# youmi-zym/TemporalStereo

Measured on AMD Instinct MI355X. Metric: stereo pairs/sec, FlyingThings3D 540x960 D=192 (aggregation hot path), higher is better.
Workload: dtype f32

## Files before the change

### include/ts_hip.h

```cpp
#ifndef TS_HIP_H
#define TS_HIP_H

#include <stddef.h>
#include <stdint.h>

#ifdef __cplusplus
extern "C" {
#endif

#define TS_OK 0
#define TS_ERR_NULL (-1)
#define TS_ERR_SHAPE (-2)
#define TS_ERR_UNSUPPORTED (-3)
#define TS_ERR_ALIGN (-4)

int ts_version(void);
const char* ts_last_error_string(void);

size_t ts_block_cost_workspace_bytes(int B, int C, int H, int W, int D, int scales);

int ts_block_cost_int_fwd(const float* left, const float* right, float* out, void* workspace,
                          int B, int C, int H, int W, int D, int scales, void* stream);

int ts_block_cost_sampled_fwd(const float* left, const float* right, const float* disp, float* out,
// ... 167 lines not shown
int ts_conv3d_hw_x6_fwd(const float* x, const void* w6, const float* scale, const float* shift, float* y,
                        int B, int Cin, int Cout, int D, int H, int W, int dilation, int act, float act_param,
                        long long in_bstride, long long in_cstride, long long out_bstride, long long out_cstride,
                        const float* addend, long long addend_bstride, void* workspace, size_t workspace_bytes, void* stream);
typedef struct ts_peer_ctx {
  void* region[8];
  int rank, world;
} ts_peer_ctx;
size_t ts_peer_region_bytes(void);
int ts_peer_max_floats(void);
int ts_peer_max_ranks(void);
int ts_peer_alloc(void** region, void* handle64);
int ts_peer_open(const void* handle64, void** region);
int ts_peer_close(void* region);
int ts_peer_free(void* region);
int ts_peer_status(const void* ctx, int* status, void* stream);
int ts_peer_status_async(const void* ctx, int* host_status, void* stream);
long long ts_peer_set_timeout_ms(long long ms);
int ts_peer_reset(const void* ctx, void* stream);
int ts_peer_all_gather(const void* ctx, const float* src, float* dst, int n, void* stream);
int ts_peer_all_reduce_sum(const void* ctx, float* buf, int n, const float* scale, void* stream);

int ts_conv3d_hw_x6s_supported(int Cin, int Cout, int H, int W, int mode);
size_t ts_conv3d_hw_x6s_weight_bytes(int Cin, int Cout, int mode);
int ts_conv3d_hw_x6s_weight_split(const float* w_t, void* w6, int Cin, int Cout, int w_pad, int mode, void* stream);
int ts_conv3d_hw_x6s_fwd(const float* x, const void* w6, const float* scale, const float* shift, float* y,
                         int B, int Cin, int Cout, int D, int H, int W, int mode, int act, float act_param,
                         long long in_bstride, long long in_cstride, long long out_bstride, long long out_cstride, void* stream);
int ts_conv3d_d_fwd(const float* x, const float* w_t, const float* scale, const float* shift, float* y,
                    int B, int Cin, int Cout, int Din, int H, int W, int k, int stride, int dilation,
                    int padding, int transposed, int act, float act_param,
                    long long in_bstride, long long in_cstride, long long out_bstride,
                    long long out_cstride, void* stream);
size_t ts_conv3d_bwd_weight_workspace_bytes(int Cin, int Cout, int taps);
int ts_conv3d_hw_bwd_data(const float* dy, const float* w_b, float* dx, int B, int Cin, int Cout, int D, int H, int W,
                          int stride, int dilation, int transposed, long long dy_bstride, long long dy_cstride,
                          long long dx_bstride, long long dx_cstride, void* stream);
int ts_conv3d_hw_bwd_weight(const float* x, const float* dy, float* dw, int B, int Cin, int Cout, int D, int H, int W,
                            int stride, int dilation, long long x_bstride, long long x_cstride, long long dy_bstride,
                            long long dy_cstride, void* workspace, size_t workspace_bytes, void* stream);
int ts_conv3d_d_bwd_data(const float* dy, const float* w_b, float* dx, int B, int Cin, int Cout, int Din, int H, int W,
                         int k, int stride, int dilation, int padding, int transposed, long long dy_bstride,
                         long long dy_cstride, long long dx_bstride, long long dx_cstride, void* stream);
int ts_conv3d_d_bwd_weight(const float* x, const float* dy, float* dw, int B, int Cin, int Cout, int Din, int H, int W,
                           int k, int stride, int dilation, int padding, long long x_bstride, long long x_cstride,
                           long long dy_bstride, long long dy_cstride, void* workspace, size_t workspace_bytes,
                           void* stream);
int ts_resize3d_add_act_fwd(const float* a, const float* add, float* out, int B, int C, int Da, int Ha, int Wa,
                            int D, int H, int W, int act, long long a_bstride, long long a_cstride,
                            long long add_bstride, long long add_cstride, long long out_bstride,
                            long long out_cstride, void* stream);
int ts_pool3d5_avgmax_fwd(const float* x, float* out_avg, float* out_max, int B, int C, int D, int H, int W,
                          long long x_bstride, long long x_cstride, long long avg_bstride, long long avg_cstride,
                          long long max_bstride, long long max_cstride, void* stream);
int ts_merge_candidates_fwd(const float* volume, const float* sample, const float* mem_sample, const float* mem_cost,
                            const float* past_w, const float* past_scale, const float* past_shift,
                            float* out_sample, float* out_volume, int B, int C, int D0, int K, int H, int W,
                            long long vol_bstride, long long vol_cstride, long long out_bstride,
                            long long out_cstride, void* stream);
int ts_convex_upsample_fwd(const float* mask, const float* disp, float* out, int B, int H, int W, int factor,
                           float disp_scale, void* stream);
int ts_convex_upsample_candidates_fwd(const float* mask, const float* disp, float* out, float* low, float* high,
                                      float* candidates, int B, int H, int W, int factor, float disp_scale, float range,
                                      int channel_offset, int channels_total, void* stream);
int ts_unet_upsample_fwd(const float* mask, const float* disp, float* out, int B, int h, int w, int Ho, int Wo,
                         void* stream);
// ... 59 lines not shown
```

### temporalstereo_amd/_lib.py

```python
import ctypes
import os
import threading

_HERE = os.path.dirname(os.path.abspath(__file__))
LIB_PATH = os.path.join(_HERE, "libts_hip.so")

_lock = threading.Lock()
_lib = None

c_f32p = ctypes.c_void_p
c_ptr = ctypes.c_void_p
c_int = ctypes.c_int
c_size = ctypes.c_size_t
c_float = ctypes.c_float

SIGNATURES = {
    "ts_version": (c_int, []),
    "ts_last_error_string": (ctypes.c_char_p, []),
    "ts_block_cost_workspace_bytes": (c_size, [c_int] * 6),
    "ts_block_cost_int_fwd": (c_int, [c_f32p, c_f32p, c_f32p, c_ptr] + [c_int] * 6 + [c_ptr]),
    "ts_block_cost_sampled_fwd": (c_int, [c_f32p, c_f32p, c_f32p, c_f32p, c_ptr] + [c_int] * 6 + [c_ptr]),
    "ts_block_cost_sampled_warped_fwd": (c_int, [c_f32p, c_f32p, c_f32p, c_f32p, c_ptr] + [c_int] * 6 + [c_ptr]),
    "ts_block_cost_sampled_corr_fwd": (c_int, [c_f32p, c_f32p, c_f32p, c_f32p, c_ptr] + [c_int] * 6 + [c_ptr]),
    "ts_conv3d_hw_warp_workspace_bytes": (c_size, [c_int] * 5),
# ... 60 lines not shown
    "ts_peer_status_async": (c_int, [c_ptr, c_ptr, c_ptr]),
    "ts_peer_set_timeout_ms": (ctypes.c_longlong, [ctypes.c_longlong]),
    "ts_peer_reset": (c_int, [c_ptr, c_ptr]),
    "ts_peer_all_gather": (c_int, [c_ptr, c_f32p, c_f32p, c_int, c_ptr]),
    "ts_peer_all_reduce_sum": (c_int, [c_ptr, c_f32p, c_int, c_f32p, c_ptr]),
    "ts_conv_weight_layout": (c_int, [c_f32p, c_f32p] + [c_int] * 4 + [ctypes.c_longlong] * 3 + [c_int, c_ptr]),
    "ts_conv_weight_layout_many": (c_int, [c_ptr, c_int, c_int, c_ptr]),
    "ts_conv_weight_layout_many2": (c_int, [c_ptr, c_int, c_int, c_ptr]),
    "ts_conv_wgrad_defer": (c_int, [c_int]),
    "ts_conv_wgrad_pending": (c_int, []),
    "ts_conv_wgrad_take": (c_int, [c_ptr, c_size, ctypes.POINTER(c_int), ctypes.POINTER(c_int)]),
    "ts_conv_wgrad_finish_many": (c_int, [c_ptr, c_int, c_int, c_ptr]),
    "ts_conv_set_chunk_cap": (c_int, [c_int]),
    "ts_conv3d_hw_x6_supported": (c_int, [c_int] * 6),
    "ts_conv3d_hw_x6_weight_bytes": (ctypes.c_size_t, [c_int] * 2),
    "ts_conv3d_hw_x6_weight_split": (c_int, [c_f32p, c_ptr, c_int, c_int, c_ptr]),
    "ts_conv3d_hw_x6_weight_split_from": (c_int, [c_f32p, c_ptr, c_int, c_int] + [ctypes.c_longlong] * 3 + [c_int, c_ptr]),
    "ts_conv3d_hw_x6_workspace_bytes": (c_size, [c_int] * 6),
    "ts_conv3d_hw_x6s_supported": (c_int, [c_int] * 5),
    "ts_conv3d_hw_x6s_weight_bytes": (c_size, [c_int] * 3),
    "ts_conv3d_hw_x6s_weight_split": (c_int, [c_f32p, c_ptr, c_int, c_int, c_int, c_int, c_ptr]),
    "ts_conv3d_hw_x6s_fwd": (c_int, [c_f32p, c_ptr, c_f32p, c_f32p, c_f32p] + [c_int] * 8 + [c_float] + [ctypes.c_longlong] * 4 + [c_ptr]),
    "ts_conv3d_hw_x6_fwd": (c_int, [c_f32p, c_ptr, c_f32p, c_f32p, c_f32p] + [c_int] * 8 + [c_float] + [ctypes.c_longlong] * 4 +
                            [c_f32p, ctypes.c_longlong, c_ptr, c_size, c_ptr]),
    "ts_conv3d_hw_fwd": (c_int, [c_f32p] * 5 + [c_int] * 10 + [c_float] + [ctypes.c_longlong] * 4 +
                         [c_f32p, ctypes.c_longlong, c_ptr, c_size, c_ptr]),
    "ts_conv3d_hw_workspace_bytes": (c_size, [c_int] * 8),
    "ts_conv3d_hw_bwd_data": (c_int, [c_f32p] * 3 + [c_int] * 9 + [ctypes.c_longlong] * 4 + [c_ptr]),
    "ts_conv3d_bwd_weight_workspace_bytes": (ctypes.c_size_t, [c_int] * 3),
    "ts_conv3d_hw_bwd_weight": (c_int, [c_f32p] * 3 + [c_int] * 8 + [ctypes.c_longlong] * 4 + [c_ptr, ctypes.c_size_t, c_ptr]),
    "ts_conv3d_d_bwd_data": (c_int, [c_f32p] * 3 + [c_int] * 11 + [ctypes.c_longlong] * 4 + [c_ptr]),
    "ts_conv3d_d_bwd_weight": (c_int, [c_f32p] * 3 + [c_int] * 10 + [ctypes.c_longlong] * 4 + [c_ptr, ctypes.c_size_t, c_ptr]),
    "ts_conv3d_d_fwd": (c_int, [c_f32p] * 5 + [c_int] * 12 + [c_float] + [ctypes.c_longlong] * 4 + [c_ptr]),
    "ts_resize3d_add_act_fwd": (c_int, [c_f32p] * 3 + [c_int] * 9 + [ctypes.c_longlong] * 6 + [c_ptr]),
    "ts_pool3d5_avgmax_fwd": (c_int, [c_f32p] * 3 + [c_int] * 5 + [ctypes.c_longlong] * 6 + [c_ptr]),
    "ts_merge_candidates_fwd": (c_int, [c_f32p] * 9 + [c_int] * 6 + [ctypes.c_longlong] * 4 + [c_ptr]),
    "ts_convex_upsample_fwd": (c_int, [c_f32p] * 3 + [c_int] * 4 + [c_float, c_ptr]),
    "ts_convex_upsample_candidates_fwd": (c_int, [c_f32p] * 6 + [c_int] * 4 + [c_float, c_float, c_int, c_int, c_ptr]),
    "ts_unet_upsample_fwd": (c_int, [c_f32p] * 3 + [c_int] * 5 + [c_ptr]),
    "ts_convex_upsample_bwd": (c_int, [c_f32p] * 5 + [c_int] * 4 + [c_float, c_ptr]),
    "ts_unet_upsample_bwd": (c_int, [c_f32p] * 5 + [c_ptr] + [c_int] * 5 + [c_ptr]),
    "ts_deconv2d_k4s2_fwd": (c_int, [c_f32p] * 5 + [c_int] * 6 + [ctypes.c_longlong, c_ptr]),
    "ts_resize_bilinear_fwd": (c_int, [c_f32p] * 2 + [c_int] * 6 + [c_float, ctypes.c_longlong, c_ptr]),
    "ts_resize_bilinear_pair_fwd": (c_int, [c_f32p] * 4 + [c_int] * 6 + [c_float, c_float, c_ptr]),
    "ts_range_candidates_fwd": (c_int, [c_f32p] * 4 + [c_int] * 3 + [c_float, c_int, c_int, c_ptr]),
    "ts_project_to_3d_fwd": (c_int, [c_f32p] * 7 + [c_int] * 6 + [c_float, c_ptr]),
    "ts_reproject_memory_workspace_bytes": (c_size, [c_int] * 5),
    "ts_reproject_memory_fwd": (c_int, [c_f32p, ctypes.c_longlong, c_int, c_int, c_f32p, c_f32p, c_int, c_f32p, c_int, c_int,
                                        c_f32p, c_int, c_f32p, c_f32p, c_f32p, c_float, c_float, c_f32p, c_f32p, c_f32p,
                                        c_ptr, c_int, c_int, c_int, c_ptr]),
    "ts_resize3d_add_act_bwd": (c_int, [c_f32p] * 5 + [c_int] * 9 + [c_ptr]),
    "ts_pool3d5_avgmax_bwd": (c_int, [c_f32p] * 4 + [c_int] * 5 + [c_ptr]),
    "ts_merge_candidates_bwd": (c_int, [c_f32p] * 5 + [c_int] * 5 + [c_ptr]),
    "ts_copy_rows_fwd": (c_int, [c_f32p] * 2 + [ctypes.c_longlong] * 4 + [c_ptr]),
    "ts_plan_create": (c_ptr, []),
    "ts_plan_destroy": (None, [c_ptr]),
    "ts_plan_length": (c_int, [c_ptr]),
    "ts_plan_add_call": (c_int, [c_ptr, ctypes.c_char_p, ctypes.POINTER(ctypes.c_ulonglong), c_int]),
    "ts_plan_run": (c_int, [c_ptr]),
    "ts_stream_fork": (c_int, [c_ptr, c_ptr]),
    "ts_event_record": (c_int, [c_int, c_ptr]),
    "ts_event_wait": (c_int, [c_int, c_ptr]),
}

_QUERIES = frozenset(n for n in SIGNATURES if n.endswith("_bytes") or n.startswith("ts_plan_") or
                     n in ("ts_version", "ts_last_error_string", "ts_conv_cout_pad", "ts_conv3d_hw_x6_supported", "ts_conv3d_hw_x6s_supported", "ts_peer_max_floats", "ts_peer_max_ranks",
                           "ts_peer_alloc", "ts_peer_open", "ts_peer_close", "ts_peer_free", "ts_peer_status", "ts_peer_status_async",
                           "ts_peer_set_timeout_ms", "ts_peer_reset", "ts_bn_set_small_elems",
                           "ts_conv_wgrad_defer", "ts_conv_wgrad_pending", "ts_conv_wgrad_take"))


def lib():
    rec = getattr(_tls, "recorder", None)
    if rec is not None:
        return rec.proxy
    return _real_lib()


def _real_lib():
    global _lib
    if _lib is None:
        with _lock:
            if _lib is None:
                if not os.path.exists(LIB_PATH):
                    raise RuntimeError(
                        "temporalstereo_amd: %s is missing -- build it with "
                        "`python -m temporalstereo_amd.build` (there is no fallback path)" % LIB_PATH)
                handle = ctypes.CDLL(LIB_PATH)
                for name, (res, args) in SIGNATURES.items():
                    fn = getattr(handle, name, None)
                    if fn is None:
                        raise RuntimeError("libts_hip.so does not export %s (stale build?)" % name)
                    fn.restype = res
                    fn.argtypes = args
                _lib = handle
    return _lib


_tls = threading.local()
# ... 105 lines not shown
```

### temporalstereo_amd/aggregation/native.py

```python
import os
import time

import torch
import torch.nn as nn

from .. import _lib
from .. import functional as TF

ACT_NONE, ACT_SILU, ACT_RELU, ACT_TANH_OFFSET, ACT_HEAD_PAIR = 0, 1, 2, 3, 4


def _stream():
    return _lib.current_stream_handle()


_PAR = {"on": False, "aux": None, "kinds": frozenset(__import__("os").environ.get("TS_BRANCHES", "hourglass").split(","))}


def _aux_stream():
    return _PAR["aux"]


_STAGE_CAP = int(os.environ.get("TS_STAGE_CHUNK_CAP", "8"))

# ... 290 lines not shown
        if getattr(f, "_tape", None) is not None:
            f._tape.splits.append((f, "x6", 0))
    return w6


X6S = os.environ.get("TS_CONV_X6S", "1") != "0"
_X6S_MIN_GRID = int(os.environ.get("TS_CONV_X6S_MIN_GRID", "256"))
_X6S_MIN_GRID_T3 = int(os.environ.get("TS_CONV_X6S_MIN_GRID_T3", "400"))
X6S_S2, X6S_T3, X6S_T4 = 0, 1, 2


def x6s_weights(f, mode):
    w6 = getattr(f, "w6s", None)
    if w6 is None:
        L = _lib._real_lib()
        w6 = torch.empty(int(L.ts_conv3d_hw_x6s_weight_bytes(f.cin, f.cout, mode)), device=f.w.device, dtype=torch.uint8)
        _lib.check(L.ts_conv3d_hw_x6s_weight_split(f.w.data_ptr(), w6.data_ptr(), f.cin, f.cout, f.w.shape[2], mode, _stream()),
                   "ts_conv3d_hw_x6s_weight_split")
        f.w6s = w6
        f.w6s_mode = mode
        if getattr(f, "_tape", None) is not None:
            f._tape.splits.append((f, "x6s", mode))
    elif getattr(f, "w6s_mode", mode) != mode:
        raise RuntimeError("x6s_weights: this layer's weights were split for mode %d, asked for mode %d" % (f.w6s_mode, mode))
    return w6


def x6s_grid(B, cout, D, H, W, mode):
    if mode == X6S_S2:
        return ((((H - 1) // 2 + 1) + 3) // 4) * ((((W - 1) // 2 + 1) + 31) // 32) * D * B * ((cout + 31) // 32)
    return ((H + 7) // 8) * ((W + 31) // 32) * D * B * ((cout + 15) // 16)


def conv_hw(x, f, stride=1, dilation=1, transposed=False, out=None, act=None, act_param=0.0, addend=None, second=None,
            out_second=None):
    B, Cin, D, H, W = x.shape
    if second is not None:
        if B != 1 or second.shape != x.shape or _strides5(second)[1] != _strides5(x)[1]:
            raise ValueError("conv_hw(second=...): two tensors of one shape and channel stride with batch 1")
        if (second.data_ptr() - x.data_ptr()) % 4:
            raise ValueError("conv_hw(second=...): allocations are not 4-byte aligned relative to each other")
        B = 2
    assert Cin == f.cin, (Cin, f.cin)
    if transposed:
        Ho, Wo = 2 * H, 2 * W
    else:
        Ho = (H + 2 * dilation - 2 * dilation - 1) // stride + 1
        Wo = (W + 2 * dilation - 2 * dilation - 1) // stride + 1
    if out is None:
        out = torch.empty((B, f.cout, D, Ho, Wo), device=x.device, dtype=torch.float32)
    ib, ic = _strides5(x)
    if second is not None:
        ib = (second.data_ptr() - x.data_ptr()) // 4
        _lib.ptr(second)
    ob, oc = _strides5(out)
    if out_second is not None:
        if second is None or out.shape[0] != 1 or out_second.shape != out.shape or _strides5(out_second)[1] != oc:
            raise ValueError("conv_hw(out_second=...): needs `second` and two outputs of one shape and channel stride")
        ob = (out_second.data_ptr() - out.data_ptr()) // 4
        _lib.ptr(out_second)
    L = _lib.lib()
    if X6 and X6S and addend is None and (stride == 2 or transposed) and dilation == 1:
        mode = X6S_T3 if transposed else X6S_S2
        if L.ts_conv3d_hw_x6s_supported(Cin, f.cout, H, W, mode) and x6s_grid(B, f.cout, D, H, W, mode) >= (_X6S_MIN_GRID_T3 if transposed else _X6S_MIN_GRID):
            rc = L.ts_conv3d_hw_x6s_fwd(_lib.ptr(x), _lib.ptr(x6s_weights(f, mode)), _lib.ptr(f.scale), _lib.ptr(f.shift), _lib.ptr(out),
                                        B, Cin, f.cout, D, H, W, mode, f.act if act is None else act, float(act_param),
                                        ib, ic, ob, oc, _stream())
            _lib.check(rc, "ts_conv3d_hw_x6s_fwd")
            return out
    wsb = int(L.ts_conv3d_hw_workspace_bytes(B, Cin, f.cout, D, H, W, stride, int(transposed)))
    x6_grid = ((H + 7) // 8) * ((W + 31) // 32) * D * B * ((f.cout + 31) // 32)
    x6_ok = X6 and L.ts_conv3d_hw_x6_supported(Cin, f.cout, W, stride, dilation, int(transposed))
    wsb6 = int(L.ts_conv3d_hw_x6_workspace_bytes(B, Cin, f.cout, D, H, W)) if x6_ok else 0
    if x6_ok and Cin < 32 and x6_grid < 512:
        x6_ok = False
    if x6_ok and (x6_grid >= _X6_MIN_GRID or wsb6 or (not wsb and x6_grid >= _X6_MIN_GRID_UNSPLIT)):
        ws6 = torch.empty(wsb6, device=x.device, dtype=torch.uint8) if wsb6 else None
        rc = L.ts_conv3d_hw_x6_fwd(_lib.ptr(x), _lib.ptr(x6_weights(f)), _lib.ptr(f.scale), _lib.ptr(f.shift), _lib.ptr(out),
                                   B, Cin, f.cout, D, H, W, dilation, f.act if act is None else act, float(act_param),
                                   ib, ic, ob, oc, _lib.ptr(addend), addend.stride(0) if addend is not None else 0, _lib.ptr(ws6), wsb6,
                                   _stream())
        _lib.check(rc, "ts_conv3d_hw_x6_fwd")
        return out
    ws = torch.empty(wsb, device=x.device, dtype=torch.uint8) if wsb else None
    rc = L.ts_conv3d_hw_fwd(_lib.ptr(x), _lib.ptr(f.w), _lib.ptr(f.scale), _lib.ptr(f.shift), _lib.ptr(out),
                            B, Cin, f.cout, D, H, W, stride, dilation, int(transposed),
                            f.act if act is None else act, float(act_param), ib, ic, ob, oc,
                            _lib.ptr(addend), addend.stride(0) if addend is not None else 0, _lib.ptr(ws), wsb, _stream())
    _lib.check(rc, "ts_conv3d_hw_fwd")
    return out


def conv_d(x, f, k, stride=1, dilation=1, padding=0, transposed=False, out=None, act=None, act_param=0.0):
    B, Cin, Din, H, W = x.shape
    assert Cin == f.cin, (Cin, f.cin)
    Dout = 2 * Din if transposed else (Din + 2 * padding - dilation * (k - 1) - 1) // stride + 1
    if out is None:
        out = torch.empty((B, f.cout, Dout, H, W), device=x.device, dtype=torch.float32)
    ib, ic = _strides5(x)
    ob, oc = _strides5(out)
    rc = _lib.lib().ts_conv3d_d_fwd(_lib.ptr(x), _lib.ptr(f.w), _lib.ptr(f.scale), _lib.ptr(f.shift), _lib.ptr(out),
                                    B, Cin, f.cout, Din, H, W, k, stride, dilation, padding, int(transposed),
                                    f.act if act is None else act, float(act_param), ib, ic, ob, oc, _stream())
    _lib.check(rc, "ts_conv3d_d_fwd")
    return out


FUSED_K1 = os.environ.get("TS_FUSED_K1", "1") != "0"


def block_cost_corr(left, right, disp, scales):
    return TF.block_cost_corr(left, right, disp, scales)


def conv_hw_warp(corr, f, q, disp, base, dilation=1):
    B, Cc, D, H, W = corr.shape
    assert Cc == f.cin, (Cc, f.cin)
    out = torch.empty((B, f.cout, D, H, W), device=corr.device, dtype=torch.float32)
    ib, ic = _strides5(corr)
    ob, oc = _strides5(out)
    wsb = TF._q("ts_conv3d_hw_warp_workspace_bytes", B, f.cout, D, H, W)
    ws = torch.empty(wsb, device=corr.device, dtype=torch.uint8)
    rc = _lib.lib().ts_conv3d_hw_warp_fwd(_lib.ptr(corr), _lib.ptr(f.w), _lib.ptr(f.scale), _lib.ptr(f.shift), _lib.ptr(out),
                                          _lib.ptr(q), _lib.ptr(disp), _lib.ptr(base), B, Cc, f.cout, D, H, W, dilation, f.act, 0.0,
                                          ib, ic, ob, oc, base.stride(0) if base is not None else 0, _lib.ptr(ws), wsb, _stream())
    _lib.check(rc, "ts_conv3d_hw_warp_fwd")
    return out


def resize_add_act(a, add, size, act=ACT_SILU):
    B, C, Da, Ha, Wa = a.shape
    D, H, W = size
    out = torch.empty((B, C, D, H, W), device=a.device, dtype=torch.float32)
    ab, ac = _strides5(a)
    bb, bc = _strides5(add) if add is not None else (0, 0)
    ob, oc = _strides5(out)
    rc = _lib.lib().ts_resize3d_add_act_fwd(_lib.ptr(a), _lib.ptr(add), _lib.ptr(out), B, C, Da, Ha, Wa, D, H, W, act,
# ... 58 lines not shown
    if 2 * C + scales * (C // 8) != f0.cin or f0.kshape != (1, 3, 3):
        raise NotImplementedError("first aggregation layer is not a (1,3,3) conv over [left | warped | corr]")
    left, rest = fold_split_input(f0, C)
    _, corr = fold_split_input(rest, C)
    q = object.__new__(Folded)
    q.cin, q.cout, q.kind, q.act, q.kshape = C, 9 * rest.cout, "d", ACT_NONE, (1, 1, 1)
    pad = int(_lib.lib().ts_conv_cout_pad(q.cout))
    q.w = torch.zeros(C, 1, pad, device=rest.w.device, dtype=torch.float32)
    q.w[:, 0, :q.cout] = rest.w[:C, :, :rest.cout].reshape(C, 9 * rest.cout)
    q.scale, q.shift = torch.ones(pad, device=q.w.device), torch.zeros(pad, device=q.w.device)
    q._tape = getattr(f0, "_tape", None)
    if q._tape is not None:
        src = getattr(f0, "src", None)
        if src is None or src[3]:
            q._tape.unsupported.append("first layer of a sampled level is itself derived")
        else:
            q._tape.layout(q.w, src[0].detach(), False, rows=(C, C), out_st=rest.cout)
    return left, rest, corr, q


class SepConv:

    def __init__(self, mod, transposed=False):
        c0, c1 = mod.conv[0], mod.conv[1]
        self.transposed = transposed
        self.f0 = fold_wrapper(c0, "hw", transposed)
        self.f1 = fold_wrapper(c1, "d", transposed)
        self.k = c1.kernel_size[0]
        self.stride, self.dil = c0.stride[1], c0.dilation[1]
        self.pad_d = c1.padding[0]
        if c0.kernel_size != (1, 3, 3) or c0.padding[1] != self.dil or c1.stride[0] != self.stride:
            raise NotImplementedError("separable conv outside the (1,3,3)+(k,1,1) family: %r" % (mod,))

    def __call__(self, x, out=None, addend=None):
        y = conv_hw(x, self.f0, self.stride, self.dil, self.transposed, addend=addend)
        return conv_d(y, self.f1, self.k, self.stride, self.dil, self.pad_d, self.transposed, out=out)


class Hourglass:

    def __init__(self, mod):
        self.c1, self.c2, self.c3, self.c4 = (SepConv(getattr(mod, n)) for n in ("conv1", "conv2", "conv3", "conv4"))
        self.c5, self.c6 = SepConv(mod.conv5, True), SepConv(mod.conv6, True)
        self.s5, self.s6 = SepConv(mod.shortcut5), SepConv(mod.shortcut6)
        self.c4.f1.act = ACT_SILU

    def __call__(self, x):
        pre = self.c2(self.c1(x))
        br = Branch("hourglass")
        with br:
            s6 = self.s6(x)
            s5 = self.s5(pre)
        out = self.c5(self.c4(self.c3(pre)))
        br.join()
        out = resize_add_act(out, s5, pre.shape[-3:])
        return resize_add_act(self.c6(out), s6, x.shape[-3:])


class Heads:

    def __init__(self, mod):
        self.delta = float(mod.delta)
        c0, self.c1 = fold_wrapper(mod.cost_head[0], "d"), fold_wrapper(mod.cost_head[1], "hw")
        o0, self.o1 = fold_wrapper(mod.off_head[0], "d"), fold_wrapper(mod.off_head[1], "hw")
        self.C = C = c0.cout
        self.co0 = fold_concat(c0, o0)
        f = object.__new__(Folded)
# ... 504 lines not shown
```

### temporalstereo_amd/csrc/plan.hip

```cpp
#include <cstdint>
#include <cstring>
#include <mutex>
#include <string>
#include <utility>
#include <vector>

#include "ts_common.hpp"

namespace {

constexpr int kMaxWords = 32;

template <class T>
T unpack(unsigned long long w) {
  static_assert(sizeof(T) <= sizeof(unsigned long long), "argument wider than a plan word");
  T v;
  std::memcpy(&v, &w, sizeof(T));
  return v;
}

template <class... A, size_t... I>
int call_with(int (*f)(A...), const unsigned long long* w, std::index_sequence<I...>) {
  return f(unpack<A>(w[I])...);
}
template <class... A>
int call_with(int (*f)(A...), const unsigned long long* w) {
  return call_with(f, w, std::index_sequence_for<A...>{});
}
template <class... A>
constexpr int arity(int (*)(A...)) { return static_cast<int>(sizeof...(A)); }

struct Entry {
  const char* name;
  int (*thunk)(const unsigned long long*);
  int nargs;
};

#define TS_PLAN_OP(fn) Entry{#fn, [](const unsigned long long* w) { return call_with(&fn, w); }, arity(&fn)}

const Entry kTable[] = {
    TS_PLAN_OP(ts_block_cost_int_fwd),      TS_PLAN_OP(ts_block_cost_sampled_fwd),
    TS_PLAN_OP(ts_block_cost_sampled_warped_fwd),
    TS_PLAN_OP(ts_block_cost_sampled_corr_fwd), TS_PLAN_OP(ts_conv3d_hw_warp_fwd),
    TS_PLAN_OP(ts_cat_fms_fwd),             TS_PLAN_OP(ts_dif_fms_fwd),             TS_PLAN_OP(ts_inverse_warp_3d_fwd),
    TS_PLAN_OP(ts_block_cost_int_bwd),      TS_PLAN_OP(ts_block_cost_sampled_bwd),
    TS_PLAN_OP(ts_topk_softargmax_fwd),     TS_PLAN_OP(ts_topk_softargmax_bwd),
    TS_PLAN_OP(ts_softargmin_fwd),          TS_PLAN_OP(ts_softargmin_bwd),
    TS_PLAN_OP(ts_argmax_select_fwd),       TS_PLAN_OP(ts_softsplat_sum_fwd),
    TS_PLAN_OP(ts_softsplat_sum_fwd_deterministic), TS_PLAN_OP(ts_softsplat_sum_bwd_input), TS_PLAN_OP(ts_softsplat_sum_bwd_flow),
    TS_PLAN_OP(ts_softsplat_softmax_fwd),   TS_PLAN_OP(ts_project_to_3d_fwd),
    TS_PLAN_OP(ts_conv3d_hw_fwd),           TS_PLAN_OP(ts_conv3d_d_fwd),
    TS_PLAN_OP(ts_conv3d_hw_bwd_data),      TS_PLAN_OP(ts_conv3d_hw_bwd_weight),
    TS_PLAN_OP(ts_conv3d_d_bwd_data),       TS_PLAN_OP(ts_conv3d_d_bwd_weight),
    TS_PLAN_OP(ts_resize3d_add_act_fwd),    TS_PLAN_OP(ts_pool3d5_avgmax_fwd),
    TS_PLAN_OP(ts_merge_candidates_fwd),    TS_PLAN_OP(ts_convex_upsample_fwd),
    TS_PLAN_OP(ts_convex_upsample_candidates_fwd),
    TS_PLAN_OP(ts_unet_upsample_fwd),       TS_PLAN_OP(ts_deconv2d_k4s2_fwd),
    TS_PLAN_OP(ts_resize_bilinear_fwd),     TS_PLAN_OP(ts_range_candidates_fwd),
    TS_PLAN_OP(ts_copy_rows_fwd),           TS_PLAN_OP(ts_stream_fork),
    TS_PLAN_OP(ts_event_record),            TS_PLAN_OP(ts_event_wait),
    TS_PLAN_OP(ts_resize3d_add_act_bwd),    TS_PLAN_OP(ts_pool3d5_avgmax_bwd),
    TS_PLAN_OP(ts_merge_candidates_bwd),
    TS_PLAN_OP(ts_reproject_memory_fwd),
    TS_PLAN_OP(ts_resize_bilinear_pair_fwd),
    TS_PLAN_OP(ts_calib_stream),             TS_PLAN_OP(ts_conv_set_chunk_cap),
    TS_PLAN_OP(ts_wasserstein_loss_fwd),     TS_PLAN_OP(ts_wasserstein_loss_bwd),
    TS_PLAN_OP(ts_disp_smooth_l1_fwd),       TS_PLAN_OP(ts_disp_smooth_l1_bwd),
    TS_PLAN_OP(ts_correlation_fwd),          TS_PLAN_OP(ts_correlation_bwd),
    TS_PLAN_OP(ts_bn_stats_fwd),             TS_PLAN_OP(ts_bn_apply_act_fwd),
    TS_PLAN_OP(ts_bn_act_bwd_reduce),        TS_PLAN_OP(ts_bn_act_bwd_apply),
    TS_PLAN_OP(ts_convex_upsample_bwd),      TS_PLAN_OP(ts_unet_upsample_bwd),
    TS_PLAN_OP(ts_conv_weight_layout),      TS_PLAN_OP(ts_conv_weight_layout_many),
    TS_PLAN_OP(ts_conv3d_hw_x6_fwd),        TS_PLAN_OP(ts_conv3d_hw_x6_weight_split), TS_PLAN_OP(ts_conv3d_hw_x6_weight_split_from),
    TS_PLAN_OP(ts_conv3d_hw_x6s_fwd),       TS_PLAN_OP(ts_conv3d_hw_x6s_weight_split),
    TS_PLAN_OP(ts_peer_all_gather),         TS_PLAN_OP(ts_peer_all_reduce_sum),
    TS_PLAN_OP(ts_bn_train_fwd),            TS_PLAN_OP(ts_bn_train_bwd),
    TS_PLAN_OP(ts_channel_splice_fwd),
    TS_PLAN_OP(ts_candidates_in_range_fwd), TS_PLAN_OP(ts_candidates_in_range_bwd),
    TS_PLAN_OP(ts_offset_head_fwd),         TS_PLAN_OP(ts_offset_head_bwd),
    TS_PLAN_OP(ts_space_to_depth2_fwd),
    TS_PLAN_OP(ts_deconv2d_k4s2_weight_to_conv3), TS_PLAN_OP(ts_deconv2d_k4s2_wgrad_from_conv3),
    TS_PLAN_OP(ts_clip_rmsprop_step),       TS_PLAN_OP(ts_bn_sync_merge),
    TS_PLAN_OP(ts_bn_fold_many),
    TS_PLAN_OP(ts_conv_weight_layout_many2), TS_PLAN_OP(ts_conv_wgrad_finish_many), TS_PLAN_OP(ts_channel_sum_fwd),
// ... 165 lines not shown
```

### temporalstereo_amd/csrc/ts_common.hpp

```cpp
#pragma once
#include <hip/hip_runtime.h>

#include <cstdarg>
#include <cstdint>
#include <cstdio>

#include "../../include/ts_hip.h"

#define TS_ABI_VERSION 10

namespace ts {

char* err_buf();
int fail(int code, const char* fmt, ...);

inline hipStream_t as_stream(void* s) { return reinterpret_cast<hipStream_t>(s); }

inline bool aligned16(const void* p) { return (reinterpret_cast<uintptr_t>(p) & 15u) == 0; }

inline size_t round_up(size_t v, size_t a) { return (v + a - 1) / a * a; }

inline int launched(const char* what) {
  hipError_t e = hipGetLastError();
  if (e != hipSuccess) return fail(static_cast<int>(e), "%s: %s", what, hipGetErrorString(e));
  return TS_OK;
}

constexpr int kWave = 64;
constexpr int kNumCU = 256;
constexpr int kNumXCD = 8;

}

#define TS_REQUIRE_PTR(p)                                                     \
  do {                                                                        \
    if ((p) == nullptr) return ts::fail(TS_ERR_NULL, "%s is NULL", #p);       \
  } while (0)
#define TS_REQUIRE_ALIGNED(p)                                                          \
  do {                                                                                 \
    if (!ts::aligned16(p)) return ts::fail(TS_ERR_ALIGN, "%s not 16-byte aligned", #p); \
  } while (0)
#define TS_REQUIRE(cond, code, ...)                       \
// ... 4 lines not shown
```

Baseline: 1462.

## Fuse separable (1,3,3)+(3,1,1) conv pair into one register-resident kernel

Adds a fused kernel that computes the spatial 3x3 conv, its BN/activation, and the following depth-3 conv for each output pixel. The intermediate tensor stays in registers, so it is never written to or read back from global memory, and one launch replaces two. Middle channels can be split across wave slices, with a shared-memory reduction to combine them. It is used only when the existing router would have picked the plain f32 path and one of the fixed channel/depth template combinations matches. The cost is heavy per-thread register use and redundant FMA work per pixel, which may lower occupancy.

```diff
diff --git a/include/ts_hip.h b/include/ts_hip.h
--- a/include/ts_hip.h
+++ b/include/ts_hip.h
@@ -223,6 +223,13 @@
                     int padding, int transposed, int act, float act_param,
                     long long in_bstride, long long in_cstride, long long out_bstride,
                     long long out_cstride, void* stream);
+int ts_conv3d_sep_supported(int B, int Cin, int Cmid, int Cout, int D, int H, int W, int k, int stride, int dilation, int pad_d,
+                            int transposed);
+int ts_conv3d_sep_fwd(const float* x, const float* w0, const float* scale0, const float* shift0, int act0, float act_param0,
+                      const float* w1, const float* scale1, const float* shift1, int act1, float act_param1, float* y,
+                      int B, int Cin, int Cmid, int Cout, int D, int H, int W, int k, int stride, int dilation, int pad_d,
+                      int transposed, long long x_bstride, long long x_cstride, long long y_bstride, long long y_cstride,
+                      void* stream);
 size_t ts_conv3d_bwd_weight_workspace_bytes(int Cin, int Cout, int taps);
 int ts_conv3d_hw_bwd_data(const float* dy, const float* w_b, float* dx, int B, int Cin, int Cout, int D, int H, int W,
                           int stride, int dilation, int transposed, long long dy_bstride, long long dy_cstride,
diff --git a/temporalstereo_amd/_lib.py b/temporalstereo_amd/_lib.py
--- a/temporalstereo_amd/_lib.py
+++ b/temporalstereo_amd/_lib.py
@@ -116,6 +116,9 @@
     "ts_conv3d_d_bwd_data": (c_int, [c_f32p] * 3 + [c_int] * 11 + [ctypes.c_longlong] * 4 + [c_ptr]),
     "ts_conv3d_d_bwd_weight": (c_int, [c_f32p] * 3 + [c_int] * 10 + [ctypes.c_longlong] * 4 + [c_ptr, ctypes.c_size_t, c_ptr]),
     "ts_conv3d_d_fwd": (c_int, [c_f32p] * 5 + [c_int] * 12 + [c_float] + [ctypes.c_longlong] * 4 + [c_ptr]),
+    "ts_conv3d_sep_supported": (c_int, [c_int] * 12),
+    "ts_conv3d_sep_fwd": (c_int, [c_f32p] * 4 + [c_int, c_float] + [c_f32p] * 3 + [c_int, c_float, c_f32p] + [c_int] * 12 +
+                          [ctypes.c_longlong] * 4 + [c_ptr]),
     "ts_resize3d_add_act_fwd": (c_int, [c_f32p] * 3 + [c_int] * 9 + [ctypes.c_longlong] * 6 + [c_ptr]),
     "ts_pool3d5_avgmax_fwd": (c_int, [c_f32p] * 3 + [c_int] * 5 + [ctypes.c_longlong] * 6 + [c_ptr]),
     "ts_merge_candidates_fwd": (c_int, [c_f32p] * 9 + [c_int] * 6 + [ctypes.c_longlong] * 4 + [c_ptr]),
@@ -148,7 +151,7 @@
 }
 
 _QUERIES = frozenset(n for n in SIGNATURES if n.endswith("_bytes") or n.startswith("ts_plan_") or
-                     n in ("ts_version", "ts_last_error_string", "ts_conv_cout_pad", "ts_conv3d_hw_x6_supported", "ts_conv3d_hw_x6s_supported", "ts_peer_max_floats", "ts_peer_max_ranks",
+                     n in ("ts_version", "ts_last_error_string", "ts_conv_cout_pad", "ts_conv3d_hw_x6_supported", "ts_conv3d_hw_x6s_supported", "ts_conv3d_sep_supported", "ts_peer_max_floats", "ts_peer_max_ranks",
                            "ts_peer_alloc", "ts_peer_open", "ts_peer_close", "ts_peer_free", "ts_peer_status", "ts_peer_status_async",
                            "ts_peer_set_timeout_ms", "ts_peer_reset", "ts_bn_set_small_elems",
                            "ts_conv_wgrad_defer", "ts_conv_wgrad_pending", "ts_conv_wgrad_take"))
diff --git a/temporalstereo_amd/aggregation/native.py b/temporalstereo_amd/aggregation/native.py
--- a/temporalstereo_amd/aggregation/native.py
+++ b/temporalstereo_amd/aggregation/native.py
@@ -346,6 +346,22 @@
     return ((H + 7) // 8) * ((W + 31) // 32) * D * B * ((cout + 15) // 16)
 
 
+def _hw_route(L, B, Cin, cout, D, H, W, stride, dilation, transposed, has_addend):
+    if X6 and X6S and not has_addend and (stride == 2 or transposed) and dilation == 1:
+        mode = X6S_T3 if transposed else X6S_S2
+        if L.ts_conv3d_hw_x6s_supported(Cin, cout, H, W, mode) and x6s_grid(B, cout, D, H, W, mode) >= (_X6S_MIN_GRID_T3 if transposed else _X6S_MIN_GRID):
+            return "x6s", mode
+    wsb = int(L.ts_conv3d_hw_workspace_bytes(B, Cin, cout, D, H, W, stride, int(transposed)))
+    x6_grid = ((H + 7) // 8) * ((W + 31) // 32) * D * B * ((cout + 31) // 32)
+    x6_ok = X6 and L.ts_conv3d_hw_x6_supported(Cin, cout, W, stride, dilation, int(transposed))
+    wsb6 = int(L.ts_conv3d_hw_x6_workspace_bytes(B, Cin, cout, D, H, W)) if x6_ok else 0
+    if x6_ok and Cin < 32 and x6_grid < 512:
+        x6_ok = False
+    if x6_ok and (x6_grid >= _X6_MIN_GRID or wsb6 or (not wsb and x6_grid >= _X6_MIN_GRID_UNSPLIT)):
+        return "x6", wsb6
+    return "f32", wsb
+
+
 def conv_hw(x, f, stride=1, dilation=1, transposed=False, out=None, act=None, act_param=0.0, addend=None, second=None,
             out_second=None):
     B, Cin, D, H, W = x.shape
@@ -374,21 +390,16 @@
         ob = (out_second.data_ptr() - out.data_ptr()) // 4
         _lib.ptr(out_second)
     L = _lib.lib()
-    if X6 and X6S and addend is None and (stride == 2 or transposed) and dilation == 1:
-        mode = X6S_T3 if transposed else X6S_S2
-        if L.ts_conv3d_hw_x6s_supported(Cin, f.cout, H, W, mode) and x6s_grid(B, f.cout, D, H, W, mode) >= (_X6S_MIN_GRID_T3 if transposed else _X6S_MIN_GRID):
-            rc = L.ts_conv3d_hw_x6s_fwd(_lib.ptr(x), _lib.ptr(x6s_weights(f, mode)), _lib.ptr(f.scale), _lib.ptr(f.shift), _lib.ptr(out),
-                                        B, Cin, f.cout, D, H, W, mode, f.act if act is None else act, float(act_param),
-                                        ib, ic, ob, oc, _stream())
-            _lib.check(rc, "ts_conv3d_hw_x6s_fwd")
-            return out
-    wsb = int(L.ts_conv3d_hw_workspace_bytes(B, Cin, f.cout, D, H, W, stride, int(transposed)))
-    x6_grid = ((H + 7) // 8) * ((W + 31) // 32) * D * B * ((f.cout + 31) // 32)
-    x6_ok = X6 and L.ts_conv3d_hw_x6_supported(Cin, f.cout, W, stride, dilation, int(transposed))
-    wsb6 = int(L.ts_conv3d_hw_x6_workspace_bytes(B, Cin, f.cout, D, H, W)) if x6_ok else 0
-    if x6_ok and Cin < 32 and x6_grid < 512:
-        x6_ok = False
-    if x6_ok and (x6_grid >= _X6_MIN_GRID or wsb6 or (not wsb and x6_grid >= _X6_MIN_GRID_UNSPLIT)):
+    route, extra = _hw_route(L, B, Cin, f.cout, D, H, W, stride, dilation, transposed, addend is not None)
+    if route == "x6s":
+        mode = extra
+        rc = L.ts_conv3d_hw_x6s_fwd(_lib.ptr(x), _lib.ptr(x6s_weights(f, mode)), _lib.ptr(f.scale), _lib.ptr(f.shift), _lib.ptr(out),
+                                    B, Cin, f.cout, D, H, W, mode, f.act if act is None else act, float(act_param),
+                                    ib, ic, ob, oc, _stream())
+        _lib.check(rc, "ts_conv3d_hw_x6s_fwd")
+        return out
+    if route == "x6":
+        wsb6 = extra
         ws6 = torch.empty(wsb6, device=x.device, dtype=torch.uint8) if wsb6 else None
         rc = L.ts_conv3d_hw_x6_fwd(_lib.ptr(x), _lib.ptr(x6_weights(f)), _lib.ptr(f.scale), _lib.ptr(f.shift), _lib.ptr(out),
                                    B, Cin, f.cout, D, H, W, dilation, f.act if act is None else act, float(act_param),
@@ -396,6 +407,7 @@
                                    _stream())
         _lib.check(rc, "ts_conv3d_hw_x6_fwd")
         return out
+    wsb = extra
     ws = torch.empty(wsb, device=x.device, dtype=torch.uint8) if wsb else None
     rc = L.ts_conv3d_hw_fwd(_lib.ptr(x), _lib.ptr(f.w), _lib.ptr(f.scale), _lib.ptr(f.shift), _lib.ptr(out),
                             B, Cin, f.cout, D, H, W, stride, dilation, int(transposed),
@@ -417,6 +429,29 @@
                                     B, Cin, f.cout, Din, H, W, k, stride, dilation, padding, int(transposed),
                                     f.act if act is None else act, float(act_param), ib, ic, ob, oc, _stream())
     _lib.check(rc, "ts_conv3d_d_fwd")
+    return out
+
+
+SEP = os.environ.get("TS_CONV_SEP", "1") != "0"
+
+
+def conv_sep(x, sc, out=None):
+    B, Cin, D, H, W = x.shape
+    f0, f1 = sc.f0, sc.f1
+    assert Cin == f0.cin and f1.cin == f0.cout, (Cin, f0.cin, f1.cin, f0.cout)
+    if sc.transposed:
+        Do, Ho, Wo = 2 * D, 2 * H, 2 * W
+    else:
+        Do, Ho, Wo = (D - 1) // sc.stride + 1, (H - 1) // sc.stride + 1, (W - 1) // sc.stride + 1
+    if out is None:
+        out = torch.empty((B, f1.cout, Do, Ho, Wo), device=x.device, dtype=torch.float32)
+    ib, ic = _strides5(x)
+    ob, oc = _strides5(out)
+    rc = _lib.lib().ts_conv3d_sep_fwd(_lib.ptr(x), _lib.ptr(f0.w), _lib.ptr(f0.scale), _lib.ptr(f0.shift), f0.act, 0.0,
+                                      _lib.ptr(f1.w), _lib.ptr(f1.scale), _lib.ptr(f1.shift), f1.act, 0.0, _lib.ptr(out),
+                                      B, Cin, f0.cout, f1.cout, D, H, W, sc.k, sc.stride, sc.dil, sc.pad_d, int(sc.transposed),
+                                      ib, ic, ob, oc, _stream())
+    _lib.check(rc, "ts_conv3d_sep_fwd")
     return out
 
 
@@ -541,7 +576,19 @@
         if c0.kernel_size != (1, 3, 3) or c0.padding[1] != self.dil or c1.stride[0] != self.stride:
             raise NotImplementedError("separable conv outside the (1,3,3)+(k,1,1) family: %r" % (mod,))
 
+    def fused(self, x, addend=None):
+        if not SEP or addend is not None:
+            return False
+        B, Cin, D, H, W = x.shape
+        L = _lib.lib()
+        if not L.ts_conv3d_sep_supported(B, Cin, self.f0.cout, self.f1.cout, D, H, W, self.k, self.stride, self.dil, self.pad_d,
+                                         int(self.transposed)):
+            return False
+        return _hw_route(L, B, Cin, self.f0.cout, D, H, W, self.stride, self.dil, self.transposed, False)[0] == "f32"
+
     def __call__(self, x, out=None, addend=None):
+        if self.fused(x, addend):
+            return conv_sep(x, self, out=out)
         y = conv_hw(x, self.f0, self.stride, self.dil, self.transposed, addend=addend)
         return conv_d(y, self.f1, self.k, self.stride, self.dil, self.pad_d, self.transposed, out=out)
 
diff --git a/temporalstereo_amd/csrc/conv_sep.hip b/temporalstereo_amd/csrc/conv_sep.hip
--- /dev/null
+++ b/temporalstereo_amd/csrc/conv_sep.hip
@@ -0,0 +1,294 @@
+#include "conv_common.hpp"
+
+namespace {
+
+enum SepMode { SEP_S1 = 0, SEP_S1D2 = 1, SEP_S2 = 2, SEP_T = 3 };
+
+typedef float f32x2 __attribute__((ext_vector_type(2)));
+
+struct SepArgs {
+  const float* x; const float* w0; const float* scale0; const float* shift0;
+  const float* w1; const float* scale1; const float* shift1; float* y;
+  int H, W, Ho, Wo;
+  int npix;
+  int act0, act1;
+  float p0, p1;
+  long long xb, xc, yb, yc;
+};
+
+template <int MODE, int D>
+struct SepGeom {
+  static constexpr bool T = MODE == SEP_T;
+  static constexpr int ST = MODE == SEP_S2 ? 2 : 1;
+  static constexpr int DL = MODE == SEP_S1D2 ? 2 : 1;
+  static constexpr int DOUT = T ? 2 * D : (ST == 2 ? (D - 1) / 2 + 1 : D);
+  static constexpr int in_plane(int od, int kd) {
+    if (T) {
+      const int n = od + 1 - kd;
+      return (n >= 0 && (n & 1) == 0 && n / 2 < D) ? n / 2 : -1;
+    }
+    const int id = od * ST - DL + kd * DL;
+    return (id >= 0 && id < D) ? id : -1;
+  }
+};
+
+template <int S, int NI>
+struct SepRed {
+  static constexpr int cap = 48 * 1024 / (S * 64 * 4);
+  static constexpr int CH = S == 1 ? 1 : (NI < cap ? NI : cap);
+  static constexpr int PHASES = (NI + CH - 1) / CH;
+  static constexpr int floats = S == 1 ? 1 : S * CH * 64;
+};
+
+template <int MODE, int CIN, int CM, int CO, int D, int S>
+__global__ void __launch_bounds__(64 * S)
+sep_pair_kernel(SepArgs a) {
+  using G = SepGeom<MODE, D>;
+  constexpr int CMS = CM / S, DOUT = G::DOUT, NI = DOUT * CO;
+  static_assert(CMS % 2 == 0 && CO % 2 == 0, "channel pairs");
+  using R = SepRed<S, NI>;
+  __shared__ float red[R::floats];
+
+  const int lane = threadIdx.x & 63;
+  const int slice = __builtin_amdgcn_readfirstlane(static_cast<int>(threadIdx.x >> 6));
+  const int p_raw = blockIdx.x * 64 + lane;
+  const bool live = p_raw < a.npix;
+  const unsigned p = static_cast<unsigned>(live ? p_raw : a.npix - 1);
+
+  int b, oy, ox, py = 0, px = 0;
+  if constexpr (G::T) {
+    const unsigned hw = static_cast<unsigned>(a.H * a.W);
+    b = static_cast<int>(p / (4u * hw));
+    const unsigned r = p - static_cast<unsigned>(b) * 4u * hw;
+    const unsigned cls = r / hw, q = r - cls * hw;
+    py = static_cast<int>(cls >> 1); px = static_cast<int>(cls & 1u);
+    const int oy2 = static_cast<int>(q / static_cast<unsigned>(a.W));
+    oy = 2 * oy2 + py; ox = 2 * static_cast<int>(q - static_cast<unsigned>(oy2) * a.W) + px;
+  } else {
+    const unsigned hw = static_cast<unsigned>(a.Ho * a.Wo);
+    b = static_cast<int>(p / hw);
+    const unsigned r = p - static_cast<unsigned>(b) * hw;
+    oy = static_cast<int>(r / static_cast<unsigned>(a.Wo)); ox = static_cast<int>(r - static_cast<unsigned>(oy) * a.Wo);
+  }
+
+  f32x2 mid[D][CMS / 2];
+#pragma unroll
+  for (int d = 0; d < D; ++d)
+#pragma unroll
+    for (int j = 0; j < CMS / 2; ++j) mid[d][j] = f32x2{0.f, 0.f};
+
+  int iy[3], ix[3];
+  bool vy[3], vx[3];
+#pragma unroll
+  for (int k = 0; k < 3; ++k) {
+    if constexpr (G::T) {
+      const int ny = oy + 1 - k, nx = ox + 1 - k;
+      iy[k] = ny >> 1; ix[k] = nx >> 1;
+      vy[k] = ((ny & 1) == 0) && ny >= 0 && iy[k] < a.H;
+      vx[k] = ((nx & 1) == 0) && nx >= 0 && ix[k] < a.W;
+    } else {
+      iy[k] = oy * G::ST + (k - 1) * G::DL; ix[k] = ox * G::ST + (k - 1) * G::DL;
+      vy[k] = iy[k] >= 0 && iy[k] < a.H;
+      vx[k] = ix[k] >= 0 && ix[k] < a.W;
+    }
+  }
+  const long long plane = static_cast<long long>(a.H) * a.W;
+  const float* xb = a.x + b * a.xb;
+  const float* w0 = a.w0 + slice * CMS;
+#pragma unroll 1
+  for (int ci = 0; ci < CIN; ++ci) {
+    const float* xc = xb + ci * a.xc;
+#pragma unroll
+    for (int ky = 0; ky < 3; ++ky) {
+#pragma unroll
+      for (int kx = 0; kx < 3; ++kx) {
+        const bool v = vy[ky] && vx[kx];
+        if constexpr (G::T) {
+          if (!v) continue;
+        }
+        const int off = v ? iy[ky] * a.W + ix[kx] : 0;
+        const float* wt = w0 + (ci * 9 + ky * 3 + kx) * CM;
+        f32x2 w[CMS / 2];
+#pragma unroll
+        for (int j = 0; j < CMS / 2; ++j) w[j] = f32x2{wt[2 * j], wt[2 * j + 1]};
+#pragma unroll
+        for (int d = 0; d < D; ++d) {
+          const float xv = v ? xc[d * plane + off] : 0.f;
+          const f32x2 xx = f32x2{xv, xv};
+#pragma unroll
+          for (int j = 0; j < CMS / 2; ++j) mid[d][j] = __builtin_elementwise_fma(xx, w[j], mid[d][j]);
+        }
+      }
+    }
+  }
+#pragma unroll
+  for (int j = 0; j < CMS / 2; ++j) {
+    const int cm = slice * CMS + 2 * j;
+    const float s0 = a.scale0[cm], s1 = a.scale0[cm + 1], h0 = a.shift0[cm], h1 = a.shift0[cm + 1];
+#pragma unroll
+    for (int d = 0; d < D; ++d) {
+      mid[d][j].x = apply_act(fmaf(mid[d][j].x, s0, h0), a.act0, a.p0);
+      mid[d][j].y = apply_act(fmaf(mid[d][j].y, s1, h1), a.act0, a.p0);
+    }
+  }
+
+  f32x2 out[DOUT][CO / 2];
+#pragma unroll
+  for (int od = 0; od < DOUT; ++od)
+#pragma unroll
+    for (int c = 0; c < CO / 2; ++c) out[od][c] = f32x2{0.f, 0.f};
+#pragma unroll
+  for (int j = 0; j < CMS; ++j) {
+#pragma unroll
+    for (int kd = 0; kd < 3; ++kd) {
+      const float* wt = a.w1 + ((slice * CMS + j) * 3 + kd) * CO;
+      f32x2 w[CO / 2];
+#pragma unroll
+      for (int c = 0; c < CO / 2; ++c) w[c] = f32x2{wt[2 * c], wt[2 * c + 1]};
+#pragma unroll
+      for (int od = 0; od < DOUT; ++od) {
+        const int id = G::in_plane(od, kd);
+        if (id < 0) continue;
+        const float m = (j & 1) ? mid[id][j >> 1].y : mid[id][j >> 1].x;
+        const f32x2 mm = f32x2{m, m};
+#pragma unroll
+        for (int c = 0; c < CO / 2; ++c) out[od][c] = __builtin_elementwise_fma(mm, w[c], out[od][c]);
+      }
+    }
+  }
+
+  const long long hwo = static_cast<long long>(a.Ho) * a.Wo;
+  float* yb = a.y + b * a.yb + static_cast<long long>(oy) * a.Wo + ox;
+  if constexpr (S == 1) {
+    if (!live) return;
+#pragma unroll
+    for (int od = 0; od < DOUT; ++od)
+#pragma unroll
+      for (int c = 0; c < CO / 2; ++c)
+#pragma unroll
+        for (int h = 0; h < 2; ++h) {
+          const int co = 2 * c + h;
+          const float v = h ? out[od][c].y : out[od][c].x;
+          yb[co * a.yc + od * hwo] = apply_act(fmaf(v, a.scale1[co], a.shift1[co]), a.act1, a.p1);
+        }
+  } else {
+#pragma unroll
+    for (int ph = 0; ph < R::PHASES; ++ph) {
+      constexpr int CH = R::CH;
+      if (ph) __syncthreads();
+#pragma unroll
+      for (int i = 0; i < CH; ++i) {
+        const int item = ph * CH + i;
+        if (item < NI) {
+          const int od = item / CO, co = item % CO;
+          red[(slice * CH + i) * 64 + lane] = (co & 1) ? out[od][co >> 1].y : out[od][co >> 1].x;
+        }
+      }
+      __syncthreads();
+      for (int i = slice; i < CH; i += S) {
+        const int item = ph * CH + i;
+        if (item >= NI) break;
+        float v = red[i * 64 + lane];
+#pragma unroll
+        for (int s = 1; s < S; ++s) v += red[(s * CH + i) * 64 + lane];
+        const int od = item / CO, co = item % CO;
+        if (live) yb[co * a.yc + od * hwo] = apply_act(fmaf(v, a.scale1[co], a.shift1[co]), a.act1, a.p1);
+      }
+    }
+  }
+}
+
+#define TS_SEP_COMBOS(X)                                                                                            \
+  X(SEP_S1, 8, 8, 8, 5) X(SEP_S1D2, 8, 8, 8, 5) X(SEP_S2, 8, 16, 16, 5) X(SEP_S1, 16, 16, 16, 3)                     \
+  X(SEP_S2, 16, 16, 16, 3) X(SEP_S1, 16, 16, 16, 2) X(SEP_T, 16, 16, 16, 2) X(SEP_T, 16, 8, 8, 3)                    \
+  X(SEP_S1, 16, 16, 16, 5) X(SEP_S1D2, 16, 16, 16, 5) X(SEP_S2, 16, 32, 32, 5) X(SEP_S1, 32, 32, 32, 3)              \
+  X(SEP_S2, 32, 32, 32, 3) X(SEP_S1, 32, 32, 32, 2) X(SEP_T, 32, 32, 32, 2) X(SEP_T, 32, 16, 16, 3)
+
+typedef void (*SepKernel)(SepArgs);
+
+template <int MODE, int CIN, int CM, int CO, int D>
+SepKernel sep_kernel_for(int S) {
+  static_assert(CM % 8 == 0, "middle channels: 8, 16, 32");
+  if (S == CM / 8) return &sep_pair_kernel<MODE, CIN, CM, CO, D, CM / 8>;
+  if constexpr (CM / 4 <= 8) if (S == CM / 4) return &sep_pair_kernel<MODE, CIN, CM, CO, D, CM / 4>;
+  if constexpr (CM / 2 <= 8) if (S == CM / 2) return &sep_pair_kernel<MODE, CIN, CM, CO, D, CM / 2>;
+  return nullptr;
+}
+
+int sep_mode(int k, int stride, int dilation, int pad_d, int transposed) {
+  if (k != 3) return -1;
+  if (transposed) return (stride == 2 && dilation == 1 && pad_d == 1) ? SEP_T : -1;
+  if (stride == 2) return (dilation == 1 && pad_d == 1) ? SEP_S2 : -1;
+  if (stride == 1 && pad_d == dilation) return dilation == 1 ? SEP_S1 : (dilation == 2 ? SEP_S1D2 : -1);
+  return -1;
+}
+
+constexpr long long kSepWaves = 256;
+int sep_slices(long long npix, int Cmid) {
+  const long long waves = (npix + 63) / 64;
+  int S = Cmid > 8 ? Cmid / 8 : 1;
+  while (S < 8 && waves * S < kSepWaves && Cmid / (2 * S) >= 2) S *= 2;
+  if (const char* e = getenv("TS_CONV_SEP_SLICES")) {
+    const int f = atoi(e);
+    if (f == 1 || f == 2 || f == 4 || f == 8) S = f;
+  }
+  return S;
+}
+
+SepKernel sep_find(int mode, int Cin, int Cmid, int Cout, int D, int S) {
+#define TS_SEP_FIND(M, CI, CMID, COUT, DD) \
+  if (mode == M && Cin == CI && Cmid == CMID && Cout == COUT && D == DD) return sep_kernel_for<M, CI, CMID, COUT, DD>(S);
+  TS_SEP_COMBOS(TS_SEP_FIND)
+#undef TS_SEP_FIND
+  return nullptr;
+}
+
+long long sep_npix(int B, int H, int W, int mode) {
+  const long long Ho = mode == SEP_T ? 2ll * H : (mode == SEP_S2 ? (H - 1) / 2 + 1 : H);
+  const long long Wo = mode == SEP_T ? 2ll * W : (mode == SEP_S2 ? (W - 1) / 2 + 1 : W);
+  return static_cast<long long>(B) * Ho * Wo;
+}
+
+}
+
+extern "C" int ts_conv3d_sep_supported(int B, int Cin, int Cmid, int Cout, int D, int H, int W, int k, int stride, int dilation,
+                                       int pad_d, int transposed) {
+  if (B <= 0 || H <= 0 || W <= 0) return 0;
+  const int mode = sep_mode(k, stride, dilation, pad_d, transposed);
+  if (mode < 0) return 0;
+  const long long npix = sep_npix(B, H, W, mode);
+  if (npix >= (1ll << 30)) return 0;
+  return sep_find(mode, Cin, Cmid, Cout, D, sep_slices(npix, Cmid)) != nullptr ? 1 : 0;
+}
+
+extern "C" int ts_conv3d_sep_fwd(const float* x, const float* w0, const float* scale0, const float* shift0, int act0, float act_param0,
+                                 const float* w1, const float* scale1, const float* shift1, int act1, float act_param1, float* y,
+                                 int B, int Cin, int Cmid, int Cout, int D, int H, int W, int k, int stride, int dilation, int pad_d,
+                                 int transposed, long long x_bstride, long long x_cstride, long long y_bstride, long long y_cstride,
+                                 void* stream) {
+  TS_REQUIRE_PTR(x); TS_REQUIRE_PTR(w0); TS_REQUIRE_PTR(scale0); TS_REQUIRE_PTR(shift0);
+  TS_REQUIRE_PTR(w1); TS_REQUIRE_PTR(scale1); TS_REQUIRE_PTR(shift1); TS_REQUIRE_PTR(y);
+  TS_REQUIRE(B > 0 && Cin > 0 && Cmid > 0 && Cout > 0 && D > 0 && H > 0 && W > 0, TS_ERR_SHAPE, "conv3d_sep: non-positive size");
+  TS_REQUIRE(act0 >= 0 && act0 <= 3 && act1 >= 0 && act1 <= 3, TS_ERR_SHAPE, "conv3d_sep: unknown activation");
+  TS_REQUIRE(x_bstride >= 0 && x_cstride >= 0 && y_bstride >= 0 && y_cstride >= 0, TS_ERR_SHAPE, "conv3d_sep: negative stride");
+  const int mode = sep_mode(k, stride, dilation, pad_d, transposed);
+  TS_REQUIRE(mode >= 0, TS_ERR_UNSUPPORTED, "conv3d_sep: k %d stride %d dilation %d padding %d transposed %d is not a fused pair", k,
+             stride, dilation, pad_d, transposed);
+  const long long npix = sep_npix(B, H, W, mode);
+  TS_REQUIRE(npix < (1ll << 30), TS_ERR_UNSUPPORTED, "conv3d_sep: too many pixels");
+  const int S = sep_slices(npix, Cmid);
+  const SepKernel kern = sep_find(mode, Cin, Cmid, Cout, D, S);
+  TS_REQUIRE(kern != nullptr, TS_ERR_UNSUPPORTED, "conv3d_sep: no instance for %d -> %d -> %d channels, D %d (ts_conv3d_sep_supported)",
+             Cin, Cmid, Cout, D);
+  SepArgs a;
+  a.x = x; a.w0 = w0; a.scale0 = scale0; a.shift0 = shift0; a.w1 = w1; a.scale1 = scale1; a.shift1 = shift1; a.y = y;
+  a.H = H; a.W = W;
+  a.Ho = static_cast<int>(mode == SEP_T ? 2 * H : (mode == SEP_S2 ? (H - 1) / 2 + 1 : H));
+  a.Wo = static_cast<int>(mode == SEP_T ? 2 * W : (mode == SEP_S2 ? (W - 1) / 2 + 1 : W));
+  a.npix = static_cast<int>(npix);
+  a.act0 = act0; a.act1 = act1; a.p0 = act_param0; a.p1 = act_param1;
+  a.xb = x_bstride; a.xc = x_cstride; a.yb = y_bstride; a.yc = y_cstride;
+  const unsigned blocks = static_cast<unsigned>((npix + 63) / 64);
+  hipLaunchKernelGGL(kern, dim3(blocks), dim3(64 * S), 0, ts::as_stream(stream), a);
+  return ts::launched("sep_pair_kernel");
+}
diff --git a/temporalstereo_amd/csrc/plan.hip b/temporalstereo_amd/csrc/plan.hip
--- a/temporalstereo_amd/csrc/plan.hip
+++ b/temporalstereo_amd/csrc/plan.hip
@@ -50,6 +50,7 @@
     TS_PLAN_OP(ts_softsplat_sum_fwd_deterministic), TS_PLAN_OP(ts_softsplat_sum_bwd_input), TS_PLAN_OP(ts_softsplat_sum_bwd_flow),
     TS_PLAN_OP(ts_softsplat_softmax_fwd),   TS_PLAN_OP(ts_project_to_3d_fwd),
     TS_PLAN_OP(ts_conv3d_hw_fwd),           TS_PLAN_OP(ts_conv3d_d_fwd),
+    TS_PLAN_OP(ts_conv3d_sep_fwd),
     TS_PLAN_OP(ts_conv3d_hw_bwd_data),      TS_PLAN_OP(ts_conv3d_hw_bwd_weight),
     TS_PLAN_OP(ts_conv3d_d_bwd_data),       TS_PLAN_OP(ts_conv3d_d_bwd_weight),
     TS_PLAN_OP(ts_resize3d_add_act_fwd),    TS_PLAN_OP(ts_pool3d5_avgmax_fwd),
diff --git a/temporalstereo_amd/csrc/ts_common.hpp b/temporalstereo_amd/csrc/ts_common.hpp
--- a/temporalstereo_amd/csrc/ts_common.hpp
+++ b/temporalstereo_amd/csrc/ts_common.hpp
@@ -7,7 +7,7 @@
 
 #include "../../include/ts_hip.h"
 
-#define TS_ABI_VERSION 10
+#define TS_ABI_VERSION 11
 
 namespace ts {
 
```

Result: slower. 1078 (median of 2 runs) (-26.3%).
